# StevenChang5/Canny_Edge

Hardware: AMD Instinct MI355X
Metric: Mpixels/s device-resident Canny (4K gray, frames in HBM, whole pipeline); % HBM roofline on Sobel+NMS in `roofline`; the end-to-end (host->host, PCIe-inclusive) rate is `end_to_end` (higher is better)
Workload: dtype f32+s16; 1 GPU; 128x 3840x2160 gray frames per GPU per step, sigma=1.4, thresholds 50/150, inputs resident in HBM; frames_per_gpu=128, height=2160, width=3840

## Files before the change

### canny_edge_amd/csrc/canny_capi.hip

```cpp
#include "canny_hip.h"
#include "canny_kernels.h"

#include <hip/hip_runtime.h>
#include <sched.h>

#include <algorithm>
#include <atomic>
#include <chrono>
#include <condition_variable>
#include <deque>
#include <memory>
#include <cmath>
#include <cstdint>
#include <cstdio>
#include <cctype>
#include <climits>
#include <cstdlib>
#include <cstring>
#include <mutex>
#include <new>
#include <string>
#include <thread>
#include <vector>
#if defined(__SSE2__)
// ... 259 lines not shown
    hipStream_t stream = nullptr;
    uint64_t *S = nullptr;
    const uint64_t *C = nullptr;
    unsigned *sched = nullptr, *flags = nullptr;
    unsigned *host = nullptr, *host_dev = nullptr;
    hipEvent_t event = nullptr;
    HystGeom g{};
    short *edges = nullptr;
    int edge_value = 0;
    int iter = 0;
    unsigned seq = 0;
    bool converged = false;
};

}

struct canny_hip_ctx {
    int device = 0;
    hipStream_t own_stream = nullptr;
    hipStream_t stream = nullptr;
    std::string last_error;
    int last_hyst_iters = 0;
    int gaussian_path = 0;
    int sobel_nms_path = 0;
    int tune_sobel_seg = 0;
    int fuse_classify = 1;
    int smoothed_u8 = 1;
    int last_canny_u8 = 0;
    int gray_rule = 0;
    int fuse_gray = 1;
    int last_fused_gray = 0;
    int hyst_tail = 1;
    int hyst_tail_after = 2;
    bool hyst_iters_async = false;
    int batch_workers = 0;
    int batch_chunk_mb = 0;
    int batch_chunk_frames = 0;
    int batch_pipe_mode = 0;
    int batch_compact = 0;
    int batch_expand_threads = 0;
    std::unique_ptr<ExpandPool> expand_pool;
    struct BatchPipe;
    std::vector<BatchPipe *> batch_pool;

    DevBuf tmp_f32;
    DevBuf smoothed;
    DevBuf edges16;
    DevBuf gray;
    DevBuf hist;
    DevBuf thr;
    DevBuf points;
    DevBuf hough_accum, hough_ws, hough_tab;
    std::vector<float> hough_tab_host;
    float hough_tab_key[3] = {0, 0, 0};
    int hough_tab_n = 0;
    int hough_path = 0;
    int hough_lds_kb = 0;
    DevBuf cc_parent, cc_ws;
    DevBuf ct_ws;
    DevBuf pg_ws, pg_points;
    DevBuf edt_cols, edt_stack;
    DevBuf seg_ws, seg_lines, seg_work;
    DevBuf circ_accum, circ_ws;
    DevBuf plane_s, plane_c, stamps, flags;
    DevBuf io[4];
    std::string ws_name;
// ... 412 lines not shown
        if ((rc = make_taps(sigma, taps))) return rc;
        const bool fuse = sm_u8 && color->fuse && gaussian_color_fusable(ctx, taps, *color, h, w);
        ctx->last_fused_gray = fuse;
        if (fuse) {
            StageTimer tm(ctx, CANNY_HIP_STAGE_GAUSSIAN);
            HIP_TRY(ctx, launch_gaussian_march_u8_color(d_img, color->ch, color->rule, (uint8_t *)sm, h, w, n, taps,
                                                        ctx->stream));
        } else {
            HIP_TRY(ctx, ctx->gray.ensure(npx(h, w, n)));
            if ((rc = dev_to_gray(ctx, d_img, *color, h, w, n, (unsigned char *)ctx->gray.p))) return rc;
            if ((rc = dev_gaussian(ctx, (const unsigned char *)ctx->gray.p, sigma, h, w, n, sm, sm_u8))) return rc;
        }
    } else {
        if (color) ctx->last_fused_gray = 0;
        if ((rc = dev_gaussian(ctx, d_img, sigma, h, w, n, sm, sm_u8))) return rc;
    }
    const int *pairs = thr ? thr->pairs : nullptr;
    if (thr && thr->rule) {
        int *out = thr->out;
        if (!out) {
            HIP_TRY(ctx, ctx->thr.ensure((size_t)n * 2 * sizeof(int)));
            out = (int *)ctx->thr.p;
        }
        HIP_TRY(ctx, ctx->hist.ensure((size_t)n * kHistBins * sizeof(uint32_t)));
        uint32_t *hist = (uint32_t *)ctx->hist.p;
        StageTimer tm(ctx, CANNY_HIP_STAGE_HYST_CLASSIFY);
        HIP_TRY(ctx, hipMemsetAsync(hist, 0, (size_t)n * kHistBins * sizeof(uint32_t), ctx->stream));
        HIP_TRY(ctx, thr->rule == kAutoMedian ? launch_hist_intensity(sm, sm_u8 != 0, hist, h, w, n, ctx->stream)
                                              : launch_hist_gradient(sm, sm_u8 != 0, hist, h, w, n, ctx->stream));
        HIP_TRY(ctx, launch_thr_select(hist, n, thr->rule, thr->low, thr->high, out, ctx->stream));
        pairs = out;
    }
    auto fused_sobel = [&](const short *smp, short *edges, uint64_t *S, uint64_t *C, const HystGeom &gg, int ev,
                           const LaunchEvents &le, const int *pp) -> hipError_t {
        return sm_u8 ? launch_sobel_nms_classify_march_u8in((const uint8_t *)smp, edges, S, C, gg, lo, hi, ev,
                                                            ctx->stream, ctx->tune_sobel_seg, le, pp)
                     : launch_sobel_nms_classify_march(smp, edges, S, C, gg, lo, hi, ev, ctx->stream,
                                                       ctx->tune_sobel_seg, le, pp);
    };
    if (fused) {
        HystGeom g = make_hyst_geom(h, w, n);
        if ((rc = ensure_hyst(ctx, g))) return rc;
        uint64_t *S = (uint64_t *)ctx->plane_s.p, *C = (uint64_t *)ctx->plane_c.p;
        const int edge_value = 255 >= hi ? 255 : 0;
        if (ctx->overlap_hysteresis && n >= 16) {
            if ((rc = ensure_aux_stream(ctx))) return rc;
            const int nA = n / 2, nB = n - nA;
            const HystGeom gA = make_hyst_geom(h, w, nA), gB = make_hyst_geom(h, w, nB);
            const size_t px_a = npx(h, w, nA);
            HIP_TRY(ctx, launch_hyst_prepare(S, C, g, true, (unsigned *)ctx->stamps.p,
                                             (unsigned *)ctx->flags.p, ctx->stream, 2));
            PropLane A = main_lane(ctx, gA, d_edges, edge_value), B = main_lane(ctx, gB, d_edges + px_a, edge_value);
            A.stream = ctx->aux_stream;
            A.event = ctx->aux_event;
            B.S += gA.words();
            B.C += gA.words();
            B.sched += hyst_sched_words(gA);
            B.flags += 2;
            B.host += 4;
            B.host_dev += 4;
            {
                StageTimer tm(ctx, CANNY_HIP_STAGE_SOBEL_NMS, nullptr, true);
                HIP_TRY(ctx, fused_sobel(sm, d_edges, A.S, (uint64_t *)A.C, gA, edge_value, tm.launch_events(), pairs));
            }
            HIP_TRY(ctx, hipEventRecord(ctx->fork_event, ctx->stream));
            HIP_TRY(ctx, hipStreamWaitEvent(ctx->aux_stream, ctx->fork_event, 0));
            ctx->last_hyst_iters = 0;
            if ((rc = lane_launch_chunk(ctx, A))) return rc;
            {
                StageTimer tm(ctx, CANNY_HIP_STAGE_SOBEL_NMS, nullptr, true);
                const short *smB = sm_u8 ? (const short *)((const uint8_t *)sm + px_a) : sm + px_a;
                HIP_TRY(ctx, fused_sobel(smB, d_edges + px_a, B.S, (uint64_t *)B.C, gB, edge_value, tm.launch_events(),
                                         pairs ? pairs + 2 * (size_t)nA : nullptr));
            }
            if ((rc = lane_launch_chunk(ctx, B))) return rc;
            for (PropLane *L : {&A, &B}) {
                if ((rc = lane_wait(ctx, *L))) return rc;
                while (!L->converged) {
                    if ((rc = lane_launch_chunk(ctx, *L)) || (rc = lane_wait(ctx, *L))) return rc;
                }
            }
            HIP_TRY(ctx, hipStreamWaitEvent(ctx->stream, A.event, 0));
            return CANNY_HIP_OK;
        }
        if ((rc = prepare_hyst(ctx, g, true))) return rc;
        {
            StageTimer tm(ctx, CANNY_HIP_STAGE_SOBEL_NMS, nullptr, true);
            HIP_TRY(ctx, fused_sobel(sm, d_edges, S, C, g, edge_value, tm.launch_events(), pairs));
        }
        if (ctx->hyst_tail && g.tiles_x * g.tiles_y <= kTailMaxTiles) {
            StageTimer tm(ctx, CANNY_HIP_STAGE_HYST_PROPAGATE);
            unsigned *sched = (unsigned *)ctx->stamps.p, *flags = (unsigned *)ctx->flags.p;
            const int wide = ctx->hyst_tail_after;
            for (int k = 0; k < wide; k++)
                HIP_TRY(ctx, launch_hyst_propagate(S, C, sched, flags, k, g, ctx->stream, d_edges, edge_value,
                                                   true));
            HIP_TRY(ctx, launch_hyst_tail(S, C, sched, flags, wide, g, ctx->stream, d_edges, edge_value));
            ctx->hyst_iters_async = true;
            return CANNY_HIP_OK;
        }
        ctx->hyst_iters_async = false;
        return run_propagation(ctx, g, false, []() -> int { return CANNY_HIP_OK; }, d_edges, edge_value);
    }
    if ((rc = dev_sobel_nms(ctx, sm, h, w, n, d_edges))) return rc;
    return dev_hysteresis(ctx, d_edges, h, w, n, lo, hi, pairs);
}

int finish_pending(canny_hip_ctx *ctx)
{
    if (!ctx->has_pend) return CANNY_HIP_OK;
    ctx->has_pend = false;
    PropLane &L = ctx->pend;
    int rc;
    if ((rc = lane_wait(ctx, L))) return rc;
    while (!L.converged)
        if ((rc = lane_launch_chunk(ctx, L)) || (rc = lane_wait(ctx, L))) return rc;
    if (L.stream != ctx->stream) HIP_TRY(ctx, hipStreamWaitEvent(ctx->stream, L.event, 0));
    return CANNY_HIP_OK;
}

int dev_canny_stream(canny_hip_ctx *ctx, const unsigned char *d_img, float sigma, int lo, int hi, int h, int w, int n,
                     short *d_edges)
{
    if (h < 2 || w < 2) return CANNY_HIP_ERR_UNSUPPORTED;
    if (hysteresis_order_dependent(lo, hi)) return CANNY_HIP_ERR_DOMAIN;
    if (!(ctx->fuse_classify && ctx->sobel_nms_path != 1 && sobel_nms_classify_supported(h, w, lo)) ||
        (ctx->hyst_tail && make_hyst_geom(h, w, n).tiles_x * make_hyst_geom(h, w, n).tiles_y <= kTailMaxTiles)) {
        int rc = finish_pending(ctx);
        return rc ? rc : dev_canny(ctx, d_img, sigma, lo, hi, h, w, n, d_edges);
    }
// ... 844 lines not shown
    for (auto &v : ctx->pending)
        for (auto &e : v) {
            (void)hipEventDestroy(e.a);
            (void)hipEventDestroy(e.b);
        }
    for (auto &e : ctx->pool) {
        (void)hipEventDestroy(e.a);
        (void)hipEventDestroy(e.b);
    }
    if (ctx->own_stream) (void)hipStreamDestroy(ctx->own_stream);
    delete ctx;
}

int canny_hip_ctx_set_stream(canny_hip_ctx *ctx, void *hip_stream)
{
    int rc = bind(ctx);
    if (rc || (rc = finish_pending(ctx))) return rc;
    ctx->stream = hip_stream ? (hipStream_t)hip_stream : ctx->own_stream;
    return CANNY_HIP_OK;
}

int canny_hip_ctx_device(const canny_hip_ctx *ctx) { return ctx ? ctx->device : -1; }

int canny_hip_ctx_get_option(const canny_hip_ctx *ctx, const char *name, int *value)
{
    if (!ctx || !name || !value) return CANNY_HIP_ERR_INVALID;
    if (!std::strcmp(name, "smoothed_u8")) *value = ctx->smoothed_u8;
    else if (!std::strcmp(name, "last_canny_smoothed_u8")) *value = ctx->last_canny_u8;
    else if (!std::strcmp(name, "gray_rule")) *value = ctx->gray_rule;
    else if (!std::strcmp(name, "fuse_gray")) *value = ctx->fuse_gray;
    else if (!std::strcmp(name, "last_canny_fused_gray")) *value = ctx->last_fused_gray;
    else if (!std::strcmp(name, "fuse_classify")) *value = ctx->fuse_classify;
    else if (!std::strcmp(name, "hysteresis_tail")) *value = ctx->hyst_tail;
    else if (!std::strcmp(name, "gaussian_path")) *value = ctx->gaussian_path;
    else if (!std::strcmp(name, "sobel_nms_path")) *value = ctx->sobel_nms_path;
    else if (!std::strcmp(name, "tune_batch_compact")) *value = ctx->batch_compact;
    else if (!std::strcmp(name, "hough_path")) *value = ctx->hough_path;
    else if (!std::strcmp(name, "tune_hough_lds_kb")) *value = ctx->hough_lds_kb;
    else if (!std::strcmp(name, "batch_expand_threads")) *value = ctx->expand_pool ? ctx->expand_pool->size() : 0;
    else return CANNY_HIP_ERR_INVALID;
    return CANNY_HIP_OK;
}

int canny_hip_ctx_set_option(canny_hip_ctx *ctx, const char *name, int value)
{
    if (!ctx || !name || value < 0) return CANNY_HIP_ERR_INVALID;
    if (!std::strcmp(name, "gaussian_path") && value <= 2) ctx->gaussian_path = value;
    else if (!std::strcmp(name, "sobel_nms_path") && value <= 2) ctx->sobel_nms_path = value;
    else if (!std::strcmp(name, "tune_sobel_seg") && value <= 4096) ctx->tune_sobel_seg = value;
    else if (!std::strcmp(name, "fuse_classify") && value <= 1) ctx->fuse_classify = value;
    else if (!std::strcmp(name, "smoothed_u8") && value <= 1) ctx->smoothed_u8 = value;
    else if (!std::strcmp(name, "gray_rule") && value <= 1) ctx->gray_rule = value;
    else if (!std::strcmp(name, "fuse_gray") && value <= 1) ctx->fuse_gray = value;
    else if (!std::strcmp(name, "hysteresis_tail") && value <= 1) ctx->hyst_tail = value;
    else if (!std::strcmp(name, "tune_hyst_tail_after") && value >= 1 && value <= 4) ctx->hyst_tail_after = value;
    else if (!std::strcmp(name, "overlap_hysteresis") && value <= 1) ctx->overlap_hysteresis = value;
    else if (!std::strcmp(name, "tune_batch_workers") && value <= 16) ctx->batch_workers = value;
    else if (!std::strcmp(name, "tune_batch_chunk_mb") && value <= 1024) ctx->batch_chunk_mb = value;
    else if (!std::strcmp(name, "tune_batch_chunk_frames") && value <= 65535) ctx->batch_chunk_frames = value;
    else if (!std::strcmp(name, "tune_batch_pipe_mode") && value <= 2) ctx->batch_pipe_mode = value;
    else if (!std::strcmp(name, "tune_batch_compact") && value <= 1) ctx->batch_compact = value;
    else if (!std::strcmp(name, "hough_path") && value <= 2) ctx->hough_path = value;
    else if (!std::strcmp(name, "tune_hough_lds_kb") && value <= kHoughLdsMax / 1024) ctx->hough_lds_kb = value;
    else if (!std::strcmp(name, "tune_batch_expand_threads") && value <= 64) {
        if (value != ctx->batch_expand_threads) ctx->expand_pool.reset();
        ctx->batch_expand_threads = value;
    }
    else if (!std::strcmp(name, "stream_overlap") && value <= 1) {
        int rc = bind(ctx);
        if (rc || (rc = finish_pending(ctx))) return rc;
        ctx->stream_overlap = value;
    } else if (!std::strcmp(name, "profile_sample_interval") && value >= 1) {
        ctx->prof_every = (unsigned)value;
        for (auto &n : ctx->prof_seen) n = 0;
    } else if (!std::strcmp(name, "profile_stage_mask")) ctx->prof_mask = value ? (unsigned)value : ~0u;
    else if (!std::strcmp(name, "tune_sobel_px") && value <= 1) sobel_nms_set_px_variant(value);
    else if (!std::strcmp(name, "tune_sobel_variant") && value <= 2) sobel_nms_set_arith_variant(value);
    else if (!std::strcmp(name, "tune_plane_stores") && value <= 1) sobel_nms_set_plane_store_variant(value);
    else if (!std::strcmp(name, "gaussian_fma_div") && value <= 1) gaussian_set_fma_div(value != 0);
    else if (!std::strcmp(name, "tune_finalize_mode") && value <= 1) hyst_set_finalize_mode(value);
    else if (!std::strcmp(name, "tune_gaussian_variant") && value <= 4) gaussian_set_march_variant(value);
    else if (!std::strcmp(name, "tune_gaussian_seg") && value <= 8192) gaussian_set_seg_target(value);
    else return CANNY_HIP_ERR_INVALID;
    return CANNY_HIP_OK;
}

int canny_hip_synchronize(canny_hip_ctx *ctx)
{
// ... 2409 lines not shown
```

### canny_edge_amd/csrc/canny_kernels.h

```cpp
#pragma once

#include <hip/hip_runtime.h>
#include <stddef.h>
#include <stdint.h>

namespace canny {

constexpr int kMaxCenter = 64;
constexpr int kMaxWindow = 2 * kMaxCenter + 1;
constexpr int kTile = 64;

struct GaussTaps {
    int center;
    float tap[kMaxWindow];
};

struct MarchCell {
    int seg, strip;
};
__host__ __device__ inline MarchCell march_cell_of(int k, int n_segs, int n_strips)
{
    MarchCell c;
#ifdef CANNY_MARCH_ROW_MAJOR
    n_segs = 0;
// ... 72 lines not shown
            c[k] = (w[i >> 2] >> (8 * (i & 3))) & 0xffu;
        }
        const uint32_t g = __umul24(c[0], r.k0) + __umul24(c[1], r.k1) + __umul24(c[2], r.k2) + r.rnd;
        out |= (g >> r.shift) << (8 * p);
    }
    return out;
}

hipError_t launch_to_gray(const uint8_t *src, int ch, const GrayRule &rule, uint8_t *gray, size_t n_px,
                          hipStream_t stream);

bool gaussian_march_color_supported(const GaussTaps &taps, int width, int ch);
hipError_t launch_gaussian_march_u8_color(const uint8_t *src, int ch, const GrayRule &rule, uint8_t *out, int height,
                                          int width, int n_frames, const GaussTaps &taps, hipStream_t stream);

hipError_t launch_xy_gradient(const int16_t *img, int16_t *gx, int16_t *gy, int height, int width, int n_frames,
                              hipStream_t stream);
hipError_t launch_sobel(const int16_t *img, int16_t *mag, int16_t *angle, int height, int width, int n_frames,
                        hipStream_t stream);
hipError_t launch_nms(const int16_t *mag, const int16_t *angle, int16_t *out, int height, int width, int n_frames,
                      hipStream_t stream);
hipError_t launch_sobel_nms(const int16_t *smoothed, int16_t *out, int height, int width, int n_frames,
                            bool domain8, hipStream_t stream);
bool sobel_nms_march_supported(int height, int width);
void sobel_nms_set_px_variant(int v);
void sobel_nms_set_arith_variant(int v);
void sobel_nms_set_plane_store_variant(int v);
struct LaunchEvents {
    hipEvent_t start = nullptr, stop = nullptr;
};
hipError_t launch_sobel_nms_march(const int16_t *smoothed, int16_t *out, int height, int width, int n_frames,
                                  hipStream_t stream, int tune_seg = 0, const LaunchEvents &ev = {});

bool sobel_nms_classify_supported(int height, int width, int min_val);
hipError_t launch_sobel_nms_classify_march(const int16_t *smoothed, int16_t *edges, uint64_t *strong, uint64_t *conn,
                                           const HystGeom &g, int min_val, int max_val, int edge_value,
                                           hipStream_t stream, int tune_seg = 0, const LaunchEvents &ev = {},
                                           const int *pairs = nullptr);

bool sobel_nms_u8_input_supported();
hipError_t launch_sobel_nms_march_u8in(const uint8_t *smoothed, int16_t *out, int height, int width, int n_frames,
                                       hipStream_t stream, int tune_seg = 0, const LaunchEvents &ev = {});
hipError_t launch_sobel_nms_classify_march_u8in(const uint8_t *smoothed, int16_t *edges, uint64_t *strong,
                                                uint64_t *conn, const HystGeom &g, int min_val, int max_val,
                                                int edge_value, hipStream_t stream, int tune_seg = 0,
                                                const LaunchEvents &ev = {}, const int *pairs = nullptr);

__host__ __device__ inline void clamp_thresholds(int &lo, int &hi)
{
    lo = lo < 1 ? 1 : (lo > 255 ? 255 : lo);
    hi = hi < lo ? lo : (hi > 255 ? 255 : hi);
}

constexpr int kAutoMedian = 1, kAutoQuantile = 2;
constexpr int kHistBins = 257;

template <class Cum>
__host__ __device__ inline int hist_quantile(const Cum &cum, double q)
{
    const double t = ceil(q * (double)cum(kHistBins - 1));
    const unsigned long long need = t < 1.0 ? 1ull : (unsigned long long)t;
    int a = 0, b = kHistBins;
    while (a < b) {
        const int m = (a + b) >> 1;
        if (cum(m) >= need)
            b = m;
        else
            a = m + 1;
    }
    return a;
}

template <class Cum>
__host__ __device__ inline void auto_thresholds(const Cum &cum, int rule, double low, double high, int &lo, int &hi)
{
    if (rule == kAutoMedian) {
        const double m = (double)hist_quantile(cum, 0.5);
        lo = (int)floor(fmin(low * m, 256.0));
        hi = (int)floor(fmin(high * m, 256.0));
    } else {
        lo = hist_quantile(cum, low);
        hi = hist_quantile(cum, high);
    }
    clamp_thresholds(lo, hi);
}

hipError_t launch_hist_intensity(const void *plane, bool in_u8, uint32_t *hist, int height, int width, int n_frames,
                                 hipStream_t stream);
hipError_t launch_hist_gradient(const void *plane, bool in_u8, uint32_t *hist, int height, int width, int n_frames,
                                hipStream_t stream);
hipError_t launch_thr_select(const uint32_t *hist, int n_frames, int rule, double low, double high, int *pairs,
                             hipStream_t stream);

hipError_t launch_hyst_classify(const int16_t *cand, uint64_t *strong, uint64_t *conn, const HystGeom &g, int min_val,
                                int max_val, unsigned *domain_flag, hipStream_t stream, const int *pairs = nullptr);
inline size_t hyst_sched_words(const HystGeom &g) { return 5 * (size_t)g.tiles() + 4 + 4 * (size_t)g.n_frames; }
hipError_t launch_hyst_prepare(uint64_t *strong, uint64_t *conn, const HystGeom &g, bool zero_pad, unsigned *sched,
                               unsigned *flags, hipStream_t stream, int n_lanes = 1);
hipError_t launch_hyst_propagate(uint64_t *strong, const uint64_t *conn, unsigned *sched, unsigned *last_change,
                                 int iter, const HystGeom &g, hipStream_t stream, int16_t *edges = nullptr,
                                 int edge_value = 0, bool frame_queues = false);
hipError_t launch_hyst_tail(uint64_t *strong, const uint64_t *conn, unsigned *sched, unsigned *last_change,
                            int first_iter, const HystGeom &g, hipStream_t stream, int16_t *edges = nullptr,
                            int edge_value = 0);
hipError_t launch_edges_to_u8(const int16_t *edges, uint8_t *out, size_t n, hipStream_t stream);
hipError_t launch_edges_to_bits(const int16_t *edges, uint8_t *bits, int height, int width, int n_frames,
                                hipStream_t stream);
hipError_t launch_hyst_publish(const unsigned *flags, unsigned *host_flags_dev, unsigned seq, hipStream_t stream);
hipError_t launch_hyst_finalize(int16_t *cand, const uint64_t *strong, const HystGeom &g, int edge_value,
                                hipStream_t stream);
void hyst_set_finalize_mode(int mode);
hipError_t launch_fep_classify(const int16_t *cand, const uint8_t *visited, uint64_t *strong, uint64_t *conn,
                               const HystGeom &g, int start, int min_val, hipStream_t stream);
hipError_t launch_fep_finalize(int16_t *cand, uint8_t *visited, const uint64_t *strong, const HystGeom &g, int start,
                               int min_val, hipStream_t stream);

__host__ __device__ inline size_t hyst_word_index(const HystGeom &g, int f, int y, int wx)
{
    return ((((size_t)f * g.tiles_y + (y >> 6)) * g.tiles_x + wx) << 6) + (y & 63);
}
#ifdef __HIPCC__
template <bool BITS>
__device__ __forceinline__ uint64_t row_word(const void *__restrict__ src, const HystGeom &g, int row_bytes, int f,
                                             int y, int k)
{
    const int left = g.width - (k << 6);
    const uint64_t mask = left >= 64 ? ~0ull : ((1ull << left) - 1ull);
    if constexpr (!BITS) {
        return static_cast<const uint64_t *>(src)[hyst_word_index(g, f, y, k)] & mask;
    } else {
        const uint8_t *row = static_cast<const uint8_t *>(src) + ((size_t)f * g.height + y) * (size_t)row_bytes +
                             (size_t)k * 8;
        const int nb = min(8, row_bytes - k * 8);
        uint64_t w = 0;
        for (int j = 0; j < nb; j++) w |= (uint64_t)(__brev((unsigned)row[j]) >> 24) << (8 * j);
        return w & mask;
    }
// ... 169 lines not shown
```

### canny_edge_amd/csrc/canny_kernels.hip

```cpp
#include "canny_kernels.h"

#include <hip/hip_ext.h>

namespace canny {

__device__ __forceinline__ uint64_t shfl_up_u64(uint64_t v)
{
    unsigned lo = (unsigned)v, hi = (unsigned)(v >> 32);
    lo = __shfl_up(lo, 1);
    hi = __shfl_up(hi, 1);
    return ((uint64_t)hi << 32) | lo;
}
__device__ __forceinline__ uint64_t shfl_down_u64(uint64_t v)
{
    unsigned lo = (unsigned)v, hi = (unsigned)(v >> 32);
    lo = __shfl_down(lo, 1);
    hi = __shfl_down(hi, 1);
    return ((uint64_t)hi << 32) | lo;
}

__device__ __forceinline__ uint64_t readlane_u64(uint64_t v, int uniform_lane)
{
    const unsigned lo = (unsigned)__builtin_amdgcn_readlane((int)(unsigned)v, uniform_lane);
    const unsigned hi = (unsigned)__builtin_amdgcn_readlane((int)(unsigned)(v >> 32), uniform_lane);
// ... 701 lines not shown
        const bool anyL = __any((chg & 1ull) != 0), anyR = __any((chg >> 63) != 0);
        const int dy = (lane == 0 || lane == 4 || lane == 5) ? -1 : ((lane == 1 || lane == 6 || lane == 7) ? 1 : 0);
        const int dx = (lane == 2 || lane == 4 || lane == 6) ? -1 : ((lane == 3 || lane == 5 || lane == 7) ? 1 : 0);
        const uint64_t facing = dy < 0 ? top64 : bot;
        const bool hit = dy == 0 ? (dx < 0 ? anyL : anyR)
                                 : (dx == 0 ? facing != 0 : (dx < 0 ? (facing & 1ull) != 0 : (facing >> 63) != 0));
        const bool there = (dy >= 0 || hasU) && (dy <= 0 || hasD) && (dx >= 0 || hasL) && (dx <= 0 || hasR);
        const bool want = lane < 8 && hit && there;
        push_tiles(want, t + dy * g.tiles_x + dx);
    }
}

__device__ __forceinline__ void note_push(unsigned *last_change, unsigned nxt)
{
    if (__hip_atomic_load(last_change, __ATOMIC_RELAXED, __HIP_MEMORY_SCOPE_AGENT) < nxt) atomicMax(last_change, nxt);
}

__device__ __forceinline__ void process_tile(int t, int lane, uint64_t *__restrict__ strong, const HystSched &sch,
                                             unsigned *__restrict__ last_change, int iter, const HystGeom &g,
                                             int16_t *__restrict__ edges, int edge_value, uint64_t c,
                                             const TileIn &in, bool to_frame = false)
{
    const unsigned nxt = (unsigned)iter + 1u;
    unsigned *q = (nxt & 1u) ? sch.queue1 : sch.queue0;
    unsigned *cnt = sch.count + nxt % 3u;
    if (to_frame) {
        const int tpf = g.tiles_x * g.tiles_y;
        const int f = t / tpf;
        q = ((nxt & 1u) ? sch.fq1 : sch.fq0) + (size_t)f * tpf;
        cnt = sch.fcount + 4 * (size_t)f + nxt % 3u;
    }
    process_tile_with(t, lane, strong, iter, g, edges, edge_value, c, in, [&](bool want, int nb) {
        push_neighbours(want, lane, sch.stamp, (unsigned)nb, (unsigned)nb, nxt, q, cnt);
        if (__any(want) && lane == 0) note_push(last_change, nxt);
    });
}

__device__ __forceinline__ void propagate_tile(int t, int lane, uint64_t *__restrict__ strong,
                                               const uint64_t *__restrict__ conn, const HystSched &sch,
                                               unsigned *__restrict__ last_change, int iter, const HystGeom &g,
                                               int16_t *__restrict__ edges, int edge_value, uint64_t c,
                                               bool to_frame = false)
{
    if (!__any(c != 0)) return;
    const TileIn in = load_tile(t, lane, strong, g, c);
    process_tile(t, lane, strong, sch, last_change, iter, g, edges, edge_value, c, in, to_frame);
}

__global__ __launch_bounds__(256) void hyst_propagate_kernel(uint64_t *__restrict__ strong,
                                                             const uint64_t *__restrict__ conn,
                                                             unsigned *__restrict__ sched_words,
                                                             unsigned *__restrict__ last_change, int iter, HystGeom g,
                                                             int16_t *__restrict__ edges, int edge_value,
                                                             int frame_groups)
{
    const int lane = threadIdx.x & 63;
    const int wave = __builtin_amdgcn_readfirstlane(blockIdx.x * 4 + (threadIdx.x >> 6));
    const int n_waves = gridDim.x * 4;
    const int tiles = g.tiles();
    const HystSched sch = make_sched(sched_words, tiles);
    if (wave == 0 && lane == 0) sch.count[(iter + 2) % 3] = 0;
    if (iter == 0) {
        for (int t0 = wave * kSweep0Tiles; t0 < tiles; t0 += n_waves * kSweep0Tiles) {
            uint64_t c[kSweep0Tiles];
#pragma unroll
            for (int k = 0; k < kSweep0Tiles; k++)
                c[k] = (t0 + k < tiles) ? conn[(size_t)(t0 + k) * kTile + lane] : 0ull;
#pragma unroll
            for (int k = 0; k < kSweep0Tiles; k++)
                propagate_tile(t0 + k, lane, strong, conn, sch, last_change, iter, g, edges, edge_value, c[k],
                               frame_groups > 0);
        }
        return;
    }
    if (frame_groups > 0) {
        const int tpf = g.tiles_x * g.tiles_y;
        const int f = (int)blockIdx.x / frame_groups, part = (int)blockIdx.x - f * frame_groups;
        unsigned *const fcount = sch.fcount + 4 * (size_t)f;
        if (part == 0 && threadIdx.x == 0) fcount[(iter + 2) % 3] = 0;
        const unsigned n = min(__hip_atomic_load(fcount + iter % 3, __ATOMIC_RELAXED, __HIP_MEMORY_SCOPE_AGENT),
                               (unsigned)tpf);
        const unsigned *q = ((iter & 1) ? sch.fq1 : sch.fq0) + (size_t)f * tpf;
        const unsigned w = (unsigned)__builtin_amdgcn_readfirstlane(part * 4 + (int)(threadIdx.x >> 6));
        for (unsigned i = w; i < n; i += (unsigned)frame_groups * 4u) {
            const int t = (int)q[i];
            propagate_tile(t, lane, strong, conn, sch, last_change, iter, g, edges, edge_value,
                           conn[(size_t)t * kTile + lane], true);
        }
        return;
    }
    const unsigned n = __hip_atomic_load(sch.count + iter % 3, __ATOMIC_RELAXED, __HIP_MEMORY_SCOPE_AGENT);
    const unsigned *q = (iter & 1) ? sch.queue1 : sch.queue0;
    for (unsigned i = (unsigned)wave; i < n; i += (unsigned)n_waves) {
        const int t = (int)q[i];
        propagate_tile(t, lane, strong, conn, sch, last_change, iter, g, edges, edge_value,
                       conn[(size_t)t * kTile + lane]);
    }
}

constexpr int kTailTiles = 4096;
__global__ __launch_bounds__(1024) void hyst_tail_kernel(uint64_t *__restrict__ strong, const uint64_t *__restrict__ conn,
                                                         unsigned *__restrict__ sched_words,
                                                         unsigned *__restrict__ last_change, int first_iter, HystGeom g,
                                                         int16_t *__restrict__ edges, int edge_value)
{
    __shared__ unsigned s_queue[2][kTailTiles];
    __shared__ unsigned s_stamp[kTailTiles];
    __shared__ unsigned s_count[2];
    __shared__ unsigned s_last;
    const int lane = threadIdx.x & 63;
    const int wave = __builtin_amdgcn_readfirstlane(threadIdx.x >> 6), n_waves = blockDim.x >> 6;
    const int f = blockIdx.x;
    const int tpf = g.tiles_x * g.tiles_y;
    const int t_base = f * tpf;
    const HystSched sch = make_sched(sched_words, g.tiles());
    int cur = first_iter & 1;
    {
        const unsigned n0 = __hip_atomic_load(sch.fcount + 4 * (size_t)f + first_iter % 3, __ATOMIC_RELAXED,
                                              __HIP_MEMORY_SCOPE_AGENT);
        const unsigned *q0 = (cur ? sch.fq1 : sch.fq0) + (size_t)t_base;
        for (unsigned i = threadIdx.x; i < n0; i += blockDim.x)
            s_queue[cur][i] = __hip_atomic_load(q0 + i, __ATOMIC_RELAXED, __HIP_MEMORY_SCOPE_AGENT) - (unsigned)t_base;
        for (int i = threadIdx.x; i < tpf; i += blockDim.x) s_stamp[i] = 0;
        if (threadIdx.x == 0) {
            s_count[cur] = n0;
            s_count[cur ^ 1] = 0;
            s_last = 0;
        }
    }
    unsigned pushed = 0;
    for (int iter = first_iter;; iter++, cur ^= 1) {
        __syncthreads();
        const unsigned n = s_count[cur];
        __syncthreads();
        if (n == 0) break;
        if (threadIdx.x == 0) s_count[cur] = 0;
        unsigned *const q_next = s_queue[cur ^ 1];
        unsigned *const n_next = &s_count[cur ^ 1];
        const unsigned nxt = (unsigned)iter + 1u;
        for (unsigned i = (unsigned)wave; i < n; i += (unsigned)n_waves) {
            const int t = t_base + (int)s_queue[cur][i];
            const uint64_t c = conn[(size_t)t * kTile + lane];
            const TileIn in = load_tile(t, lane, strong, g);
            if (!__any(c != 0)) continue;
            process_tile_with(t, lane, strong, iter, g, edges, edge_value, c, in, [&](bool want, int nb) {
                const unsigned loc = (unsigned)(nb - t_base);
                push_neighbours(want, lane, s_stamp, loc, loc, nxt, q_next, n_next);
                if (__any(want)) pushed = nxt;
            });
        }
    }
    if (lane == 0 && pushed != 0) atomicMax(&s_last, pushed);
    __syncthreads();
    if (threadIdx.x == 0 && s_last != 0) atomicMax(last_change, s_last);
}

__global__ __launch_bounds__(256) void hyst_finalize_kernel(int16_t *__restrict__ cand,
                                                            const uint64_t *__restrict__ strong, HystGeom g,
                                                            int edge_value)
{
// ... 295 lines not shown
            for (int k = 0; k < 8; k++)
                if (k < left && px[k] != 0) byte |= 0x80u >> k;
        }
        out[b] = (uint8_t)byte;
    }
}

hipError_t launch_edges_to_bits(const int16_t *edges, uint8_t *bits, int height, int width, int n_frames,
                                hipStream_t stream)
{
    const int row_bytes = (width + 7) / 8;
    const size_t n_bytes = (size_t)n_frames * (size_t)height * (size_t)row_bytes;
    if (n_bytes == 0) return hipSuccess;
    const int vec_ok = (width % 8 == 0) && (((uintptr_t)edges & 15u) == 0);
    hipLaunchKernelGGL(edges_to_bits_kernel, dim3(grid_for(n_bytes, 256)), dim3(256), 0, stream, edges, bits, width,
                       row_bytes, n_bytes, vec_ok);
    return hipGetLastError();
}

__global__ void hyst_publish_kernel(const unsigned *__restrict__ flags, unsigned *host, unsigned seq)
{
    __hip_atomic_store(&host[0], flags[0], __ATOMIC_RELAXED, __HIP_MEMORY_SCOPE_SYSTEM);
    __hip_atomic_store(&host[1], flags[1], __ATOMIC_RELAXED, __HIP_MEMORY_SCOPE_SYSTEM);
    __hip_atomic_store(&host[2], seq, __ATOMIC_RELEASE, __HIP_MEMORY_SCOPE_SYSTEM);
}

hipError_t launch_hyst_publish(const unsigned *flags, unsigned *host_flags_dev, unsigned seq, hipStream_t stream)
{
    hipLaunchKernelGGL(hyst_publish_kernel, dim3(1), dim3(1), 0, stream, flags, host_flags_dev, seq);
    return hipGetLastError();
}

hipError_t launch_hyst_tail(uint64_t *strong, const uint64_t *conn, unsigned *sched, unsigned *last_change,
                            int first_iter, const HystGeom &g, hipStream_t stream, int16_t *edges, int edge_value)
{
    if (g.n_frames < 1 || first_iter < 1 || g.tiles_x * g.tiles_y > kTailTiles) return hipErrorInvalidValue;
    const int tpf = g.tiles_x * g.tiles_y;
    const unsigned threads = tpf >= 256 ? 1024u : (tpf >= 64 ? 512u : 256u);
    hipLaunchKernelGGL(hyst_tail_kernel, dim3((unsigned)g.n_frames), dim3(threads), 0, stream, strong, conn, sched,
                       last_change, first_iter, g, edges, edge_value);
    return hipGetLastError();
}

hipError_t launch_hyst_propagate(uint64_t *strong, const uint64_t *conn, unsigned *stamp, unsigned *last_change,
                                 int iter, const HystGeom &g, hipStream_t stream, int16_t *edges, int edge_value,
                                 bool frame_queues)
{
    if (frame_queues && (g.n_frames < 1 || g.tiles_x * g.tiles_y > kTailTiles)) return hipErrorInvalidValue;
    unsigned blocks = (unsigned)((g.tiles() + 4 * kSweep0Tiles - 1) / (4 * kSweep0Tiles));
    int frame_groups = frame_queues ? 1 : 0;
    if (iter > 0) {
        const unsigned want = (unsigned)((g.tiles() + 15) / 16);
        blocks = want < 8u ? 8u : (want > 1024u ? 1024u : want);
        if (frame_queues) {
            frame_groups = (int)(blocks / (unsigned)g.n_frames);
            if (frame_groups < 1) frame_groups = 1;
            blocks = (unsigned)frame_groups * (unsigned)g.n_frames;
        }
    }
    hipLaunchKernelGGL(hyst_propagate_kernel, dim3(blocks), dim3(256), 0, stream, strong, conn, stamp, last_change,
                       iter, g, edges, edge_value, frame_groups);
    return hipGetLastError();
}
__global__ __launch_bounds__(256) void hyst_finalize_rows_kernel(int16_t *__restrict__ cand,
                                                                 const uint8_t *__restrict__ strong, HystGeom g,
                                                                 int edge_value, int groups_per_row)
{
    const uint32_t ev = (uint32_t)(uint16_t)edge_value;
    const int chunk = (int)blockIdx.x * 4 + (int)(threadIdx.x >> 6);
    const int gx = chunk * 64 + (int)(threadIdx.x & 63);
    if (gx >= groups_per_row) return;
    const int f = (int)blockIdx.z;
    const int x0 = gx * 8;
    const size_t tile_col = ((size_t)f * g.tiles_y) * g.tiles_x + (gx >> 3);
    unsigned b[4];
#pragma unroll
    for (int k = 0; k < 4; k++) {
        const int y = (int)blockIdx.y * 4 + k;
        b[k] = 0;
        if (y < g.height)
            b[k] = strong[((tile_col + (size_t)(y >> 6) * g.tiles_x) << 9) + (size_t)(y & 63) * 8 + (gx & 7)];
    }
#pragma unroll
    for (int k = 0; k < 4; k++) {
        const int y = (int)blockIdx.y * 4 + k;
        if (y >= g.height) break;
        const uint32_t t = b[k] | (b[k] << 15);
        uint4 v;
        v.x = __umul24(t & 0x00010001u, ev);
        v.y = __umul24((t >> 2) & 0x00010001u, ev);
        v.z = __umul24((t >> 4) & 0x00010001u, ev);
        v.w = __umul24((t >> 6) & 0x00010001u, ev);
        __builtin_memcpy(cand + ((size_t)f * g.height + y) * g.width + x0, &v, 16);
    }
// ... 80 lines not shown
```

### canny_edge_amd/csrc/canny_sobel_nms_march.hip

```cpp
#include "canny_kernels.h"

#include <hip/hip_ext.h>

#include <type_traits>

namespace canny {

namespace {

typedef short s16x2 __attribute__((ext_vector_type(2)));

__device__ __forceinline__ s16x2 as_v(uint32_t u) { return __builtin_bit_cast(s16x2, u); }
__device__ __forceinline__ uint32_t as_u(s16x2 v) { return __builtin_bit_cast(uint32_t, v); }
__device__ __forceinline__ uint32_t pk_add(uint32_t a, uint32_t b) { return as_u(as_v(a) + as_v(b)); }
__device__ __forceinline__ uint32_t pk_sub(uint32_t a, uint32_t b) { return as_u(as_v(a) - as_v(b)); }
__device__ __forceinline__ uint32_t pk_mad2(uint32_t a, uint32_t b)
{
    uint32_t r;
    const uint32_t two = 0x00020002u;
    asm("v_pk_mad_i16 %0, %1, %2, %3" : "=v"(r) : "v"(a), "s"(two), "v"(b));
    return r;
}

__device__ __forceinline__ uint32_t from_left(uint32_t v)
// ... 780 lines not shown
        int mag, bin;
        if (form == 1) {
            mag = pk_pixel_mag(gx, gy, Ah, nh);
            float P, Q;
            pk_pixel_disc(gx, gy, Ah, nh, P, Q);
            bin = pk_nms_select(P, Q, 0, 45, 90, 135);
        } else {
            const int m = f_pixel_mag_word(gx, gy, Ah, nh);
            mag = form == 3 ? f_pixel_mag_store<true>(m, skip) : f_pixel_mag_store<false>(m, skip);
            float qm, qp;
            f_pixel_bin_signs(gx, gy, Ah, nh, qm, qp);
            bin = f_nms_select(f_pixel_carrier(qm, qp), 0, 45, 90, 135);
        }
        mags[i] = (int16_t)((mag >> 16) ? -1 : mag);
        bins[i] = (uint8_t)bin;
    }
}

}

hipError_t launch_selftest_sobel_pixel(int form, int lim, int16_t *mags, uint8_t *bins, hipStream_t stream)
{
    if (form < 1 || form > 3 || lim < 0 || lim > 1020) return hipErrorInvalidValue;
    const size_t total = (size_t)(2 * lim + 1) * (2 * lim + 1);
    hipLaunchKernelGGL(selftest_sobel_pixel_kernel, dim3((unsigned)((total + 255) / 256)), dim3(256), 0, stream, form,
                       lim, mags, bins);
    return hipGetLastError();
}

struct PlaneArgs {
    uint8_t *conn, *strong;
    int tiles_x, tiles_y, lo1, hi1, edge_value;
    const int *thr;
};

template <bool PLANES, int NP, bool LDS_PLANES, bool IN_U8 = false, bool FLT = false, bool THR = false>
__global__ __launch_bounds__(SNM_WPB * 64) __attribute__((amdgpu_waves_per_eu(FLT ? FLT_WAVES : 1)))
void sobel_nms_march_kernel(const void *__restrict__ in,
                                                                       int16_t *__restrict__ out, int H, int W,
                                                                       int n_strips, int n_segs, int seg_rows,
                                                                       int total_waves, PlaneArgs pl)
{
    __shared__ __attribute__((aligned(8))) uint8_t stage_lds[LDS_PLANES ? SNM_WPB * 2 * SNM_STAGE_ROWS * 72 : 8];
    uint8_t *stage_mem = stage_lds + (LDS_PLANES ? (threadIdx.x >> 6) * (2 * SNM_STAGE_ROWS * 72) : 0);
    __shared__ uint4 edge_lut[LDS_PLANES ? 256 : 1];
    if (LDS_PLANES) {
        static_assert(SNM_WPB * 64 == 256, "one table entry per thread");
        const unsigned b = threadIdx.x, ev = (unsigned)pl.edge_value;
        uint4 v;
        v.x = ((b >> 0) & 1u) * ev | (((b >> 1) & 1u) * ev) << 16;
        v.y = ((b >> 2) & 1u) * ev | (((b >> 3) & 1u) * ev) << 16;
        v.z = ((b >> 4) & 1u) * ev | (((b >> 5) & 1u) * ev) << 16;
        v.w = ((b >> 6) & 1u) * ev | (((b >> 7) & 1u) * ev) << 16;
        edge_lut[b] = v;
        __syncthreads();
    }
    unsigned bid = blockIdx.x;
    {
        const unsigned q = gridDim.x / 8u, r = gridDim.x % 8u, xcd = bid % 8u;
        bid = (xcd < r ? xcd * (q + 1u) : r * (q + 1u) + (xcd - r) * q) + bid / 8u;
    }
    const int wave = __builtin_amdgcn_readfirstlane(bid * SNM_WPB + (threadIdx.x >> 6));
    if (wave >= total_waves) return;
    const int f = wave / (n_strips * n_segs);
    const MarchCell cell = march_cell_of(wave - f * (n_strips * n_segs), n_segs, n_strips);
    const int s = cell.strip, g = cell.seg;
    StripJob jb;
    jb.lane = threadIdx.x & 63;
    jb.H = H;
    jb.W = W;
    jb.ybeg = g * seg_rows;
    jb.yend = min(H, jb.ybeg + seg_rows);
    jb.x0 = s * SnmCfg<NP>::SW + (jb.lane - 1) * SnmCfg<NP>::PX;
    jb.fin = (const int16_t *)in + (size_t)f * H * W;
    jb.fin8 = (const uint8_t *)in + (size_t)f * H * W;
    jb.fout = out + (size_t)f * H * W;
    if (PLANES) {
        jb.edge_value = pl.edge_value;
// ... 100 lines not shown
                     n_strips, n_segs, seg, (int)waves, pl);
    else if (in_u8)
        launch_timed(sobel_nms_march_kernel<false, 4, false, true>, grid, block, stream, ev, smoothed, out, height,
                     width, n_strips, n_segs, seg, (int)waves, pl);
    else if (planes && np == 4 && plane_store_variant == 0)
        launch_timed(sobel_nms_march_kernel<true, 4, true, false, false, THR>, grid, block, stream, ev, smoothed, out, height, width,
                     n_strips, n_segs, seg, (int)waves, pl);
    else if (planes && np == 4)
        launch_timed(sobel_nms_march_kernel<true, 4, false, false, false, THR>, grid, block, stream, ev, smoothed, out, height, width,
                     n_strips, n_segs, seg, (int)waves, pl);
    else if (planes)
        launch_timed(sobel_nms_march_kernel<true, 2, false, false, false, THR>, grid, block, stream, ev, smoothed, out, height, width,
                     n_strips, n_segs, seg, (int)waves, pl);
    else if (np == 4)
        launch_timed(sobel_nms_march_kernel<false, 4, false>, grid, block, stream, ev, smoothed, out, height, width,
                     n_strips, n_segs, seg, (int)waves, pl);
    else
        launch_timed(sobel_nms_march_kernel<false, 2, false>, grid, block, stream, ev, smoothed, out, height, width,
                     n_strips, n_segs, seg, (int)waves, pl);
    return hipGetLastError();
}

hipError_t launch_sobel_nms_march(const int16_t *smoothed, int16_t *out, int height, int width, int n_frames,
                                  hipStream_t stream, int tune_seg, const LaunchEvents &ev)
{
    return launch_march(smoothed, out, nullptr, height, width, n_frames, stream, tune_seg, ev);
}

bool sobel_nms_classify_supported(int height, int width, int min_val)
{
    return sobel_nms_march_supported(height, width) && width % 8 == 0 && min_val >= 1;
}

bool sobel_nms_u8_input_supported() { return px_variant == 0 && plane_store_variant == 0; }

hipError_t launch_sobel_nms_march_u8in(const uint8_t *smoothed, int16_t *out, int height, int width, int n_frames,
                                       hipStream_t stream, int tune_seg, const LaunchEvents &ev)
{
    return launch_march(smoothed, out, nullptr, height, width, n_frames, stream, tune_seg, ev, true);
}

static hipError_t classify_march_any(const void *smoothed, bool in_u8, int16_t *edges, uint64_t *strong, uint64_t *conn,
                                     const HystGeom &g, int min_val, int max_val, int edge_value, hipStream_t stream,
                                     int tune_seg, const LaunchEvents &ev, const int *pairs);

hipError_t launch_sobel_nms_classify_march(const int16_t *smoothed, int16_t *edges, uint64_t *strong, uint64_t *conn,
                                           const HystGeom &g, int min_val, int max_val, int edge_value,
                                           hipStream_t stream, int tune_seg, const LaunchEvents &ev, const int *pairs)
{
    return classify_march_any(smoothed, false, edges, strong, conn, g, min_val, max_val, edge_value, stream, tune_seg, ev,
                              pairs);
}

hipError_t launch_sobel_nms_classify_march_u8in(const uint8_t *smoothed, int16_t *edges, uint64_t *strong,
                                                uint64_t *conn, const HystGeom &g, int min_val, int max_val,
                                                int edge_value, hipStream_t stream, int tune_seg,
                                                const LaunchEvents &ev, const int *pairs)
{
    return classify_march_any(smoothed, true, edges, strong, conn, g, min_val, max_val, edge_value, stream, tune_seg, ev,
                              pairs);
}

static hipError_t classify_march_any(const void *smoothed, bool in_u8, int16_t *edges, uint64_t *strong, uint64_t *conn,
                                     const HystGeom &g, int min_val, int max_val, int edge_value, hipStream_t stream,
                                     int tune_seg, const LaunchEvents &ev, const int *pairs)
{
    if (pairs) min_val = max_val = 255;
    if (!sobel_nms_classify_supported(g.height, g.width, min_val)) return hipErrorNotSupported;
    if (edge_value < 0 || edge_value > 32767) return hipErrorInvalidValue;
    const int lo = min_val > 4096 ? 4096 : min_val;
    const int hi = max_val > 4096 ? 4096 : max_val;
    PlaneArgs pl;
    pl.conn = (uint8_t *)conn;
    pl.strong = (uint8_t *)strong;
    pl.tiles_x = g.tiles_x;
    pl.tiles_y = g.tiles_y;
    pl.lo1 = lo - 1;
    pl.hi1 = (hi > lo ? hi : lo) - 1;
    pl.edge_value = edge_value;
    pl.thr = pairs;
    if (pairs) {
        if (edge_value != 255) return hipErrorInvalidValue;
        return launch_march<true>(smoothed, edges, &pl, g.height, g.width, g.n_frames, stream, tune_seg, ev, in_u8);
    }
    return launch_march(smoothed, edges, &pl, g.height, g.width, g.n_frames, stream, tune_seg, ev, in_u8);
}

}
```

Baseline: 577,300 Mpixels/s.

## Fold hysteresis state clearing into Sobel/NMS kernel and tune propagate launch

Removes the separate hyst_prepare launch on the tail route. The fused Sobel/NMS/classify kernel now zeroes the schedule words, the flags and the padded plane rows and columns itself. Also adds seeding of the tail kernel's last-change state from per-frame counters, which lets the first propagate passes skip last_change writes. Adds a waves_per_eu=8 variant of the propagate kernel and an optional walker count for frame groups. The risk is correctness: other blocks must not read the cleared state before it is reset, and the clear loop adds strided writes to every Sobel block.

```diff
diff --git a/canny_edge_amd/csrc/canny_capi.hip b/canny_edge_amd/csrc/canny_capi.hip
--- a/canny_edge_amd/csrc/canny_capi.hip
+++ b/canny_edge_amd/csrc/canny_capi.hip
@@ -315,6 +315,10 @@
     int last_fused_gray = 0;
     int hyst_tail = 1;
     int hyst_tail_after = 2;
+    int hyst_self_clear = 1;
+    int hyst_walkers = 0;
+    int hyst_seed_last = 1;
+    int hyst_waves8 = 1;
     bool hyst_iters_async = false;
     int batch_workers = 0;
     int batch_chunk_mb = 0;
@@ -793,11 +797,11 @@
         pairs = out;
     }
     auto fused_sobel = [&](const short *smp, short *edges, uint64_t *S, uint64_t *C, const HystGeom &gg, int ev,
-                           const LaunchEvents &le, const int *pp) -> hipError_t {
+                           const LaunchEvents &le, const int *pp, const HystClear &clear = {}) -> hipError_t {
         return sm_u8 ? launch_sobel_nms_classify_march_u8in((const uint8_t *)smp, edges, S, C, gg, lo, hi, ev,
-                                                            ctx->stream, ctx->tune_sobel_seg, le, pp)
+                                                            ctx->stream, ctx->tune_sobel_seg, le, pp, clear)
                      : launch_sobel_nms_classify_march(smp, edges, S, C, gg, lo, hi, ev, ctx->stream,
-                                                       ctx->tune_sobel_seg, le, pp);
+                                                       ctx->tune_sobel_seg, le, pp, clear);
     };
     if (fused) {
         HystGeom g = make_hyst_geom(h, w, n);
@@ -844,19 +848,28 @@
             HIP_TRY(ctx, hipStreamWaitEvent(ctx->stream, A.event, 0));
             return CANNY_HIP_OK;
         }
-        if ((rc = prepare_hyst(ctx, g, true))) return rc;
+        const bool tail_route = ctx->hyst_tail && g.tiles_x * g.tiles_y <= kTailMaxTiles;
+        HystClear clear;
+        if (tail_route && ctx->hyst_self_clear && sobel_nms_classify_can_clear(g)) {
+            clear.sched = (unsigned *)ctx->stamps.p;
+            clear.flags = (unsigned *)ctx->flags.p;
+        } else if ((rc = prepare_hyst(ctx, g, true))) {
+            return rc;
+        }
         {
             StageTimer tm(ctx, CANNY_HIP_STAGE_SOBEL_NMS, nullptr, true);
-            HIP_TRY(ctx, fused_sobel(sm, d_edges, S, C, g, edge_value, tm.launch_events(), pairs));
-        }
-        if (ctx->hyst_tail && g.tiles_x * g.tiles_y <= kTailMaxTiles) {
+            HIP_TRY(ctx, fused_sobel(sm, d_edges, S, C, g, edge_value, tm.launch_events(), pairs, clear));
+        }
+        if (tail_route) {
             StageTimer tm(ctx, CANNY_HIP_STAGE_HYST_PROPAGATE);
             unsigned *sched = (unsigned *)ctx->stamps.p, *flags = (unsigned *)ctx->flags.p;
             const int wide = ctx->hyst_tail_after;
+            const bool seed = ctx->hyst_seed_last && wide <= kHystTailSeedMaxIter;
             for (int k = 0; k < wide; k++)
-                HIP_TRY(ctx, launch_hyst_propagate(S, C, sched, flags, k, g, ctx->stream, d_edges, edge_value,
-                                                   true));
-            HIP_TRY(ctx, launch_hyst_tail(S, C, sched, flags, wide, g, ctx->stream, d_edges, edge_value));
+                HIP_TRY(ctx, launch_hyst_propagate(S, C, sched, seed ? nullptr : flags, k, g, ctx->stream, d_edges,
+                                                   edge_value, true, ctx->hyst_walkers,
+                                                   ctx->hyst_waves8 != 0));
+            HIP_TRY(ctx, launch_hyst_tail(S, C, sched, flags, wide, g, ctx->stream, d_edges, edge_value, seed));
             ctx->hyst_iters_async = true;
             return CANNY_HIP_OK;
         }
@@ -1767,6 +1780,10 @@
     else if (!std::strcmp(name, "last_canny_fused_gray")) *value = ctx->last_fused_gray;
     else if (!std::strcmp(name, "fuse_classify")) *value = ctx->fuse_classify;
     else if (!std::strcmp(name, "hysteresis_tail")) *value = ctx->hyst_tail;
+    else if (!std::strcmp(name, "tune_hyst_self_clear")) *value = ctx->hyst_self_clear;
+    else if (!std::strcmp(name, "tune_hyst_walkers")) *value = ctx->hyst_walkers;
+    else if (!std::strcmp(name, "tune_hyst_seed_last")) *value = ctx->hyst_seed_last;
+    else if (!std::strcmp(name, "tune_hyst_waves8")) *value = ctx->hyst_waves8;
     else if (!std::strcmp(name, "gaussian_path")) *value = ctx->gaussian_path;
     else if (!std::strcmp(name, "sobel_nms_path")) *value = ctx->sobel_nms_path;
     else if (!std::strcmp(name, "tune_batch_compact")) *value = ctx->batch_compact;
@@ -1789,6 +1806,10 @@
     else if (!std::strcmp(name, "fuse_gray") && value <= 1) ctx->fuse_gray = value;
     else if (!std::strcmp(name, "hysteresis_tail") && value <= 1) ctx->hyst_tail = value;
     else if (!std::strcmp(name, "tune_hyst_tail_after") && value >= 1 && value <= 4) ctx->hyst_tail_after = value;
+    else if (!std::strcmp(name, "tune_hyst_self_clear") && value <= 1) ctx->hyst_self_clear = value;
+    else if (!std::strcmp(name, "tune_hyst_walkers") && value <= kHystWalkersMax) ctx->hyst_walkers = value;
+    else if (!std::strcmp(name, "tune_hyst_seed_last") && value <= 1) ctx->hyst_seed_last = value;
+    else if (!std::strcmp(name, "tune_hyst_waves8") && value <= 1) ctx->hyst_waves8 = value;
     else if (!std::strcmp(name, "overlap_hysteresis") && value <= 1) ctx->overlap_hysteresis = value;
     else if (!std::strcmp(name, "tune_batch_workers") && value <= 16) ctx->batch_workers = value;
     else if (!std::strcmp(name, "tune_batch_chunk_mb") && value <= 1024) ctx->batch_chunk_mb = value;
diff --git a/canny_edge_amd/csrc/canny_kernels.h b/canny_edge_amd/csrc/canny_kernels.h
--- a/canny_edge_amd/csrc/canny_kernels.h
+++ b/canny_edge_amd/csrc/canny_kernels.h
@@ -128,11 +128,15 @@
 hipError_t launch_sobel_nms_march(const int16_t *smoothed, int16_t *out, int height, int width, int n_frames,
                                   hipStream_t stream, int tune_seg = 0, const LaunchEvents &ev = {});
 
+struct HystClear {
+    unsigned *sched = nullptr, *flags = nullptr;
+};
 bool sobel_nms_classify_supported(int height, int width, int min_val);
+bool sobel_nms_classify_can_clear(const HystGeom &g);
 hipError_t launch_sobel_nms_classify_march(const int16_t *smoothed, int16_t *edges, uint64_t *strong, uint64_t *conn,
                                            const HystGeom &g, int min_val, int max_val, int edge_value,
                                            hipStream_t stream, int tune_seg = 0, const LaunchEvents &ev = {},
-                                           const int *pairs = nullptr);
+                                           const int *pairs = nullptr, const HystClear &clear = {});
 
 bool sobel_nms_u8_input_supported();
 hipError_t launch_sobel_nms_march_u8in(const uint8_t *smoothed, int16_t *out, int height, int width, int n_frames,
@@ -140,7 +144,8 @@
 hipError_t launch_sobel_nms_classify_march_u8in(const uint8_t *smoothed, int16_t *edges, uint64_t *strong,
                                                 uint64_t *conn, const HystGeom &g, int min_val, int max_val,
                                                 int edge_value, hipStream_t stream, int tune_seg = 0,
-                                                const LaunchEvents &ev = {}, const int *pairs = nullptr);
+                                                const LaunchEvents &ev = {}, const int *pairs = nullptr,
+                                                const HystClear &clear = {});
 
 __host__ __device__ inline void clamp_thresholds(int &lo, int &hi)
 {
@@ -193,12 +198,14 @@
 inline size_t hyst_sched_words(const HystGeom &g) { return 5 * (size_t)g.tiles() + 4 + 4 * (size_t)g.n_frames; }
 hipError_t launch_hyst_prepare(uint64_t *strong, uint64_t *conn, const HystGeom &g, bool zero_pad, unsigned *sched,
                                unsigned *flags, hipStream_t stream, int n_lanes = 1);
+constexpr int kHystWalkersMax = 64;
+constexpr int kHystTailSeedMaxIter = 2;
 hipError_t launch_hyst_propagate(uint64_t *strong, const uint64_t *conn, unsigned *sched, unsigned *last_change,
                                  int iter, const HystGeom &g, hipStream_t stream, int16_t *edges = nullptr,
-                                 int edge_value = 0, bool frame_queues = false);
+                                 int edge_value = 0, bool frame_queues = false, int walkers = 0, bool waves8 = false);
 hipError_t launch_hyst_tail(uint64_t *strong, const uint64_t *conn, unsigned *sched, unsigned *last_change,
                             int first_iter, const HystGeom &g, hipStream_t stream, int16_t *edges = nullptr,
-                            int edge_value = 0);
+                            int edge_value = 0, bool seed_last = false);
 hipError_t launch_edges_to_u8(const int16_t *edges, uint8_t *out, size_t n, hipStream_t stream);
 hipError_t launch_edges_to_bits(const int16_t *edges, uint8_t *bits, int height, int width, int n_frames,
                                 hipStream_t stream);
diff --git a/canny_edge_amd/csrc/canny_kernels.hip b/canny_edge_amd/csrc/canny_kernels.hip
--- a/canny_edge_amd/csrc/canny_kernels.hip
+++ b/canny_edge_amd/csrc/canny_kernels.hip
@@ -757,7 +757,7 @@
     }
     process_tile_with(t, lane, strong, iter, g, edges, edge_value, c, in, [&](bool want, int nb) {
         push_neighbours(want, lane, sch.stamp, (unsigned)nb, (unsigned)nb, nxt, q, cnt);
-        if (__any(want) && lane == 0) note_push(last_change, nxt);
+        if (last_change && __any(want) && lane == 0) note_push(last_change, nxt);
     });
 }
 
@@ -772,7 +772,9 @@
     process_tile(t, lane, strong, sch, last_change, iter, g, edges, edge_value, c, in, to_frame);
 }
 
-__global__ __launch_bounds__(256) void hyst_propagate_kernel(uint64_t *__restrict__ strong,
+template <bool W8>
+__global__ __launch_bounds__(256) __attribute__((amdgpu_waves_per_eu(W8 ? 8 : 1)))
+void hyst_propagate_kernel(uint64_t *__restrict__ strong,
                                                              const uint64_t *__restrict__ conn,
                                                              unsigned *__restrict__ sched_words,
                                                              unsigned *__restrict__ last_change, int iter, HystGeom g,
@@ -824,10 +826,11 @@
 }
 
 constexpr int kTailTiles = 4096;
+constexpr unsigned kWalkBlocks = 1024, kWalkBlocksForced = 16384;
 __global__ __launch_bounds__(1024) void hyst_tail_kernel(uint64_t *__restrict__ strong, const uint64_t *__restrict__ conn,
                                                          unsigned *__restrict__ sched_words,
                                                          unsigned *__restrict__ last_change, int first_iter, HystGeom g,
-                                                         int16_t *__restrict__ edges, int edge_value)
+                                                         int16_t *__restrict__ edges, int edge_value, int seed_last)
 {
     __shared__ unsigned s_queue[2][kTailTiles];
     __shared__ unsigned s_stamp[kTailTiles];
@@ -850,7 +853,13 @@
         if (threadIdx.x == 0) {
             s_count[cur] = n0;
             s_count[cur ^ 1] = 0;
-            s_last = 0;
+            unsigned last = 0;
+            if (seed_last)
+                for (int k = 1; k <= first_iter; k++)
+                    if (__hip_atomic_load(sch.fcount + 4 * (size_t)f + k % 3, __ATOMIC_RELAXED,
+                                          __HIP_MEMORY_SCOPE_AGENT) != 0)
+                        last = (unsigned)k;
+            s_last = last;
         }
     }
     unsigned pushed = 0;
@@ -1212,34 +1221,44 @@
 }
 
 hipError_t launch_hyst_tail(uint64_t *strong, const uint64_t *conn, unsigned *sched, unsigned *last_change,
-                            int first_iter, const HystGeom &g, hipStream_t stream, int16_t *edges, int edge_value)
+                            int first_iter, const HystGeom &g, hipStream_t stream, int16_t *edges, int edge_value,
+                            bool seed_last)
 {
     if (g.n_frames < 1 || first_iter < 1 || g.tiles_x * g.tiles_y > kTailTiles) return hipErrorInvalidValue;
+    if (seed_last && first_iter > kHystTailSeedMaxIter) return hipErrorInvalidValue;
     const int tpf = g.tiles_x * g.tiles_y;
     const unsigned threads = tpf >= 256 ? 1024u : (tpf >= 64 ? 512u : 256u);
     hipLaunchKernelGGL(hyst_tail_kernel, dim3((unsigned)g.n_frames), dim3(threads), 0, stream, strong, conn, sched,
-                       last_change, first_iter, g, edges, edge_value);
+                       last_change, first_iter, g, edges, edge_value, seed_last ? 1 : 0);
     return hipGetLastError();
 }
 
 hipError_t launch_hyst_propagate(uint64_t *strong, const uint64_t *conn, unsigned *stamp, unsigned *last_change,
                                  int iter, const HystGeom &g, hipStream_t stream, int16_t *edges, int edge_value,
-                                 bool frame_queues)
+                                 bool frame_queues, int walkers, bool waves8)
 {
     if (frame_queues && (g.n_frames < 1 || g.tiles_x * g.tiles_y > kTailTiles)) return hipErrorInvalidValue;
+    if (!frame_queues && !last_change) return hipErrorInvalidValue;
+    if (walkers < 0 || walkers > kHystWalkersMax) return hipErrorInvalidValue;
     unsigned blocks = (unsigned)((g.tiles() + 4 * kSweep0Tiles - 1) / (4 * kSweep0Tiles));
     int frame_groups = frame_queues ? 1 : 0;
     if (iter > 0) {
         const unsigned want = (unsigned)((g.tiles() + 15) / 16);
-        blocks = want < 8u ? 8u : (want > 1024u ? 1024u : want);
+        blocks = want < 8u ? 8u : (want > kWalkBlocks ? kWalkBlocks : want);
         if (frame_queues) {
             frame_groups = (int)(blocks / (unsigned)g.n_frames);
+            if (walkers > 0)
+                frame_groups = std::min(walkers, std::max(1, (int)(kWalkBlocksForced / (unsigned)g.n_frames)));
             if (frame_groups < 1) frame_groups = 1;
             blocks = (unsigned)frame_groups * (unsigned)g.n_frames;
         }
     }
-    hipLaunchKernelGGL(hyst_propagate_kernel, dim3(blocks), dim3(256), 0, stream, strong, conn, stamp, last_change,
-                       iter, g, edges, edge_value, frame_groups);
+    if (waves8)
+        hipLaunchKernelGGL(hyst_propagate_kernel<true>, dim3(blocks), dim3(256), 0, stream, strong, conn, stamp,
+                           last_change, iter, g, edges, edge_value, frame_groups);
+    else
+        hipLaunchKernelGGL(hyst_propagate_kernel<false>, dim3(blocks), dim3(256), 0, stream, strong, conn, stamp,
+                           last_change, iter, g, edges, edge_value, frame_groups);
     return hipGetLastError();
 }
 __global__ __launch_bounds__(256) void hyst_finalize_rows_kernel(int16_t *__restrict__ cand,
diff --git a/canny_edge_amd/csrc/canny_sobel_nms_march.hip b/canny_edge_amd/csrc/canny_sobel_nms_march.hip
--- a/canny_edge_amd/csrc/canny_sobel_nms_march.hip
+++ b/canny_edge_amd/csrc/canny_sobel_nms_march.hip
@@ -836,7 +836,35 @@
     uint8_t *conn, *strong;
     int tiles_x, tiles_y, lo1, hi1, edge_value;
     const int *thr;
+    unsigned *sched, *flags;
+    unsigned n_sched, pad_items;
 };
+
+__device__ __forceinline__ void clear_hyst_state(const PlaneArgs &pl, int H, int W)
+{
+    if (!pl.sched) return;
+    const size_t tid = (size_t)blockIdx.x * blockDim.x + threadIdx.x, stride = (size_t)gridDim.x * blockDim.x;
+    for (size_t i = tid; i < pl.n_sched; i += stride) pl.sched[i] = 0u;
+    if (tid < 2) pl.flags[tid] = 0u;
+    const unsigned per_frame = (unsigned)(pl.tiles_x + pl.tiles_y) * 64u;
+    uint64_t *const strong = (uint64_t *)pl.strong, *const conn = (uint64_t *)pl.conn;
+    for (size_t i = tid; i < pl.pad_items; i += stride) {
+        const unsigned f = (unsigned)i / per_frame, r = (unsigned)i - f * per_frame;
+        const int k = (int)(r >> 6), lane = (int)(r & 63u);
+        const int tx = k < pl.tiles_x ? k : pl.tiles_x - 1;
+        const int ty = k < pl.tiles_x ? pl.tiles_y - 1 : k - pl.tiles_x;
+        const size_t w = ((((size_t)f * pl.tiles_y + ty) * pl.tiles_x + tx) << 6) + lane;
+        const int y = ty * 64 + lane;
+        const int valid_px = min(64, W - tx * 64);
+        if (y >= H) {
+            strong[w] = 0;
+            conn[w] = 0;
+        } else if (valid_px < 64) {
+            uint8_t *sb = (uint8_t *)(strong + w), *cb = (uint8_t *)(conn + w);
+            for (int b = valid_px / 8; b < 8; b++) sb[b] = cb[b] = 0;
+        }
+    }
+}
 
 template <bool PLANES, int NP, bool LDS_PLANES, bool IN_U8 = false, bool FLT = false, bool THR = false>
 __global__ __launch_bounds__(SNM_WPB * 64) __attribute__((amdgpu_waves_per_eu(FLT ? FLT_WAVES : 1)))
@@ -848,6 +876,7 @@
     __shared__ __attribute__((aligned(8))) uint8_t stage_lds[LDS_PLANES ? SNM_WPB * 2 * SNM_STAGE_ROWS * 72 : 8];
     uint8_t *stage_mem = stage_lds + (LDS_PLANES ? (threadIdx.x >> 6) * (2 * SNM_STAGE_ROWS * 72) : 0);
     __shared__ uint4 edge_lut[LDS_PLANES ? 256 : 1];
+    if constexpr (PLANES) clear_hyst_state(pl, H, W);
     if (LDS_PLANES) {
         static_assert(SNM_WPB * 64 == 256, "one table entry per thread");
         const unsigned b = threadIdx.x, ev = (unsigned)pl.edge_value;
@@ -1014,6 +1043,12 @@
     return sobel_nms_march_supported(height, width) && width % 8 == 0 && min_val >= 1;
 }
 
+bool sobel_nms_classify_can_clear(const HystGeom &g)
+{
+    return g.n_frames >= 1 && hyst_sched_words(g) <= 0xffffffffull &&
+           64ull * (unsigned long long)(g.tiles_x + g.tiles_y) * (unsigned long long)g.n_frames <= 0xffffffffull;
+}
+
 bool sobel_nms_u8_input_supported() { return px_variant == 0 && plane_store_variant == 0; }
 
 hipError_t launch_sobel_nms_march_u8in(const uint8_t *smoothed, int16_t *out, int height, int width, int n_frames,
@@ -1024,28 +1059,29 @@
 
 static hipError_t classify_march_any(const void *smoothed, bool in_u8, int16_t *edges, uint64_t *strong, uint64_t *conn,
                                      const HystGeom &g, int min_val, int max_val, int edge_value, hipStream_t stream,
-                                     int tune_seg, const LaunchEvents &ev, const int *pairs);
+                                     int tune_seg, const LaunchEvents &ev, const int *pairs, const HystClear &clear);
 
 hipError_t launch_sobel_nms_classify_march(const int16_t *smoothed, int16_t *edges, uint64_t *strong, uint64_t *conn,
                                            const HystGeom &g, int min_val, int max_val, int edge_value,
-                                           hipStream_t stream, int tune_seg, const LaunchEvents &ev, const int *pairs)
+                                           hipStream_t stream, int tune_seg, const LaunchEvents &ev, const int *pairs,
+                                           const HystClear &clear)
 {
     return classify_march_any(smoothed, false, edges, strong, conn, g, min_val, max_val, edge_value, stream, tune_seg, ev,
-                              pairs);
+                              pairs, clear);
 }
 
 hipError_t launch_sobel_nms_classify_march_u8in(const uint8_t *smoothed, int16_t *edges, uint64_t *strong,
                                                 uint64_t *conn, const HystGeom &g, int min_val, int max_val,
                                                 int edge_value, hipStream_t stream, int tune_seg,
-                                                const LaunchEvents &ev, const int *pairs)
+                                                const LaunchEvents &ev, const int *pairs, const HystClear &clear)
 {
     return classify_march_any(smoothed, true, edges, strong, conn, g, min_val, max_val, edge_value, stream, tune_seg, ev,
-                              pairs);
+                              pairs, clear);
 }
 
 static hipError_t classify_march_any(const void *smoothed, bool in_u8, int16_t *edges, uint64_t *strong, uint64_t *conn,
                                      const HystGeom &g, int min_val, int max_val, int edge_value, hipStream_t stream,
-                                     int tune_seg, const LaunchEvents &ev, const int *pairs)
+                                     int tune_seg, const LaunchEvents &ev, const int *pairs, const HystClear &clear)
 {
     if (pairs) min_val = max_val = 255;
     if (!sobel_nms_classify_supported(g.height, g.width, min_val)) return hipErrorNotSupported;
@@ -1061,6 +1097,16 @@
     pl.hi1 = (hi > lo ? hi : lo) - 1;
     pl.edge_value = edge_value;
     pl.thr = pairs;
+    pl.sched = pl.flags = nullptr;
+    pl.n_sched = pl.pad_items = 0;
+    if (clear.sched) {
+        if (!clear.flags || !sobel_nms_classify_can_clear(g)) return hipErrorInvalidValue;
+        pl.sched = clear.sched;
+        pl.flags = clear.flags;
+        pl.n_sched = (unsigned)hyst_sched_words(g);
+        if (g.height % kTile != 0 || g.width % kTile != 0)
+            pl.pad_items = (unsigned)(64ull * (unsigned)(g.tiles_x + g.tiles_y) * (unsigned)g.n_frames);
+    }
     if (pairs) {
         if (edge_value != 255) return hipErrorInvalidValue;
         return launch_march<true>(smoothed, edges, &pl, g.height, g.width, g.n_frames, stream, tune_seg, ev, in_u8);
```

Measured after the change: 581,800 Mpixels/s, median of 6. No clear change (+0.8%).
